# scverse/squidpy

Measured on AMD Instinct MI355X. Metric: nhood_enrichment permutations/sec (1e6 spots x 30 clusters), higher is better.
Workload: dtype u8 labels / u32 counts / i64 moments; 1 GPU; nhood_enrichment: 1000000 spots (1000x1000 hex grid, nnz=5992002), 30 clusters, 10000 permutations per step per GPU, on-device Philox-keyed label shuffles; collective=none

## Files before the change

squidpy_amd/csrc/sqgr_rng.h:

```cpp
#pragma once

#include <hip/hip_runtime.h>

#include <cstdint>

namespace sqgr {

constexpr uint32_t PHILOX_M0 = 0xD2511F53u, PHILOX_M1 = 0xCD9E8D57u;
constexpr uint32_t PHILOX_W0 = 0x9E3779B9u, PHILOX_W1 = 0xBB67AE85u;
constexpr uint32_t FEISTEL_C1 = 0x88B5u, FEISTEL_C2 = 0xDB2Du;
#ifndef SQGR_FEISTEL_ROUNDS
#define SQGR_FEISTEL_ROUNDS 8
#endif
constexpr int FEISTEL_ROUNDS = SQGR_FEISTEL_ROUNDS;

__host__ __device__ inline void philox4x32_10(uint32_t c[4], uint32_t k0, uint32_t k1) {
#pragma unroll
    for (int r = 0; r < 10; ++r) {
        uint64_t p0 = (uint64_t)PHILOX_M0 * c[0];
        uint64_t p1 = (uint64_t)PHILOX_M1 * c[2];
        uint32_t n0 = (uint32_t)(p1 >> 32) ^ c[1] ^ k0;
        uint32_t n1 = (uint32_t)p1;
        uint32_t n2 = (uint32_t)(p0 >> 32) ^ c[3] ^ k1;
        uint32_t n3 = (uint32_t)p0;
// ... 55 lines not shown
}

__host__ __device__ inline FeistelDomain make_domain(uint32_t n) {
    FeistelDomain d;
    d.n = n;
    const uint32_t r = isqrt_ceil(n);
    uint32_t a = 16u;
    while (a < r) a <<= 1;
    d.A = a;
    uint32_t b = (n + d.A - 1) / d.A;
    d.B = b < 16u ? 16u : b;
    uint32_t m = 1u;
    while (m < d.B) m <<= 1;
    d.Bmask = m - 1u;
    d.ash = 16u;
    for (uint32_t t = d.A; t > 1u; t >>= 1) --d.ash;
    d.bsh = 16u;
    for (uint32_t t = m; t > 1u; t >>= 1) --d.bsh;
    return d;
}

template <int NP>
__device__ __forceinline__ void feistel_rounds(u16x2 (&a)[NP], u16x2 (&b)[NP], const FeistelDomain& d,
                                               const uint32_t* const (&pk)[NP]) {
    const u16x2 am = (u16x2)((unsigned short)(d.A - 1u));
    const u16x2 ash = (u16x2)((unsigned short)d.ash), bsh = (u16x2)((unsigned short)d.bsh);
    const u16x2 BB = (u16x2)((unsigned short)d.B);
#pragma unroll
    for (int r = 0; r < FEISTEL_ROUNDS; r += 2) {
#pragma unroll
        for (int i = 0; i < NP; ++i) {
            const u16x2 k0 = __builtin_bit_cast(u16x2, pk[i][r]);
            a[i] = (a[i] + feistel_F2(b[i], k0, ash)) & am;
        }
#pragma unroll
        for (int i = 0; i < NP; ++i) {
            const u16x2 k1 = __builtin_bit_cast(u16x2, pk[i][r + 1]);
            u16x2 t = b[i] + feistel_F2(a[i], k1, bsh);
            t = __builtin_elementwise_min(t, (u16x2)(t - BB));
            b[i] = __builtin_elementwise_min(t, (u16x2)(t - BB));
        }
    }
}

template <int NP>
__device__ __forceinline__ void sigma_rounds(u16x2 (&a)[NP], u16x2 (&b)[NP], const FeistelDomain& d,
                                             const uint32_t* const (&pk)[NP]) {
    const u16x2 am = (u16x2)((unsigned short)(d.A - 1u));
    const u16x2 ash = (u16x2)((unsigned short)d.ash), bsh = (u16x2)((unsigned short)d.bsh);
    const u16x2 BB = (u16x2)((unsigned short)d.B);
#pragma unroll
    for (int i = 0; i < NP; ++i) {
        const u16x2 k0 = __builtin_bit_cast(u16x2, pk[i][0]);
        u16x2 t = b[i] + feistel_F2(a[i], k0, bsh);
        t = __builtin_elementwise_min(t, (u16x2)(t - BB));
        b[i] = __builtin_elementwise_min(t, (u16x2)(t - BB));
    }
#pragma unroll
    for (int i = 0; i < NP; ++i) {
        const u16x2 k1 = __builtin_bit_cast(u16x2, pk[i][1]);
        a[i] = (a[i] + feistel_F2(b[i], k1, ash)) & am;
    }
}

__host__ __device__ inline uint32_t grouped_perm(uint32_t x, const FeistelDomain& d, const uint32_t* gk, const uint32_t* sk) {
    uint32_t a = x / d.B, b = x - a * d.B;
    do {
        for (int r = 0; r < FEISTEL_ROUNDS; r += 2) {
            a = (a + feistel_F1(b, gk[r], d.ash)) & (d.A - 1u);
            uint32_t t = b + feistel_F1(a, gk[r + 1], d.bsh);
            t = t >= d.B ? t - d.B : t;
            b = t >= d.B ? t - d.B : t;
        }
    } while (a * d.B + b >= d.n);
    do {
        uint32_t t = b + feistel_F1(a, sk[0], d.bsh);
        t = t >= d.B ? t - d.B : t;
        b = t >= d.B ? t - d.B : t;
        a = (a + feistel_F1(b, sk[1], d.ash)) & (d.A - 1u);
    } while (a * d.B + b >= d.n);
    return a * d.B + b;
}

__host__ __device__ inline uint32_t feistel_perm(uint32_t x, const FeistelDomain& d, const uint32_t* rk) {
    uint32_t a = x / d.B, b = x - a * d.B;
    do {
        for (int r = 0; r < FEISTEL_ROUNDS; r += 2) {
            a = (a + feistel_F1(b, rk[r], d.ash)) & (d.A - 1u);
            uint32_t t = b + feistel_F1(a, rk[r + 1], d.bsh);
            t = t >= d.B ? t - d.B : t;
            b = t >= d.B ? t - d.B : t;
        }
        x = a * d.B + b;
    } while (x >= d.n);
    return x;
}

}
```

squidpy_amd/csrc/sqgr_shuffle.h:

```cpp
#pragma once
#include "sqgr_common.h"
#include "sqgr_pcg.h"
#include "sqgr_rng.h"

namespace sqgr {

__host__ __device__ constexpr int key_words_per_row(int B, int n_libs) {
    return n_libs * ((B / FEISTEL_GROUP) * 8 + (B / 2) * 2) < (B / 2) * 8 ? (B / 2) * 8 : n_libs * ((B / FEISTEL_GROUP) * 8 + (B / 2) * 2);
}

struct LibDom {
    FeistelDomain dom;
    uint32_t aoff;
};

__device__ __forceinline__ void slab_store16(uint8_t* __restrict__ batch_base, int64_t n, int64_t i, int pw, uint32_t w0, uint32_t w1,
                                             uint32_t w2, uint32_t w3) {
    if (pw == 16) {
        *reinterpret_cast<uint4*>(batch_base + (size_t)i * 16) = make_uint4(w0, w1, w2, w3);
    } else if (pw == 8) {
        *reinterpret_cast<uint2*>(batch_base + (size_t)i * 8) = make_uint2(w0, w1);
        *reinterpret_cast<uint2*>(batch_base + (size_t)n * 8 + (size_t)i * 8) = make_uint2(w2, w3);
    } else if (pw == 4) {
        uint32_t* d = reinterpret_cast<uint32_t*>(batch_base) + i;
        d[0] = w0; d[(size_t)n] = w1; d[(size_t)2 * n] = w2; d[(size_t)3 * n] = w3;
    } else if (pw == 2) {
        uint16_t* d = reinterpret_cast<uint16_t*>(batch_base) + i;
        const uint32_t w[4] = {w0, w1, w2, w3};
#pragma unroll
        for (int q = 0; q < 8; ++q) d[(size_t)q * n] = (uint16_t)(w[q >> 1] >> (16 * (q & 1)));
    } else {
        uint8_t* d = batch_base + i;
        const uint32_t w[4] = {w0, w1, w2, w3};
#pragma unroll
        for (int q = 0; q < 16; ++q) d[(size_t)q * n] = (uint8_t)(w[q >> 2] >> (8 * (q & 3)));
    }
}

int check_labels(const int32_t* labels, int64_t n, int K, bool allow_negative);

struct LabelShuffler {
    sqgr_ctx* ctx = nullptr;
    int64_t n = 0;
    int K = 0;
    int n_libs = 1;
    bool has_libs = false;
    LibDom dom0{};
    int blk_words = 0;
    DevBuf<uint32_t> cum;
    int kpad = 0;
    bool tab_lds = true;
    DevBuf<int32_t> lib_of, rank_of;
    DevBuf<LibDom> libs;
    DevBuf<uint8_t> base_pos;
    DevBuf<uint16_t> base16;
    DevBuf<int32_t> perm_idx;
    DevBuf<uint32_t> lib_off;
    DevBuf<int32_t> spot_of;
    PcgWorkspace pcg_ws;
    bool has_labels = false;
    int max_label_count = 0;
    bool wide() const { return K > 256; }
    bool mapped() const { return spot_of.p != nullptr; }

    static int create(sqgr_ctx* ctx, int64_t n, const int32_t* labels, int K, const int32_t* lib_ids, int n_libs, LabelShuffler* out);
    int independent_mode(int B, bool* independent) const;
    int keygen(const char* timer, uint64_t seed, int64_t perm0, int nrows, int B, bool independent, uint32_t* keys, hipStream_t st) const;
    int launch_shuffle_raw(int B, int nb, const uint32_t* keys, uint8_t* slab, hipStream_t st, bool independent, int pw = 16) const;
    int gather_labels16(const char* timer, int nb, int64_t p0, int64_t p_valid, uint16_t* slab16, hipStream_t st) const;
};

int label_shuffler_create(sqgr_ctx* ctx, int64_t n, const int32_t* labels, int K, LabelShuffler** out);
void label_shuffler_destroy(LabelShuffler* s);

int label_shuffler_philox(LabelShuffler* s, uint64_t seed, int64_t perm0, int nb, uint32_t* keys_ws, uint8_t* slab, hipStream_t st);

int label_shuffler_pcg64(LabelShuffler* s, const uint64_t* states_dev, int64_t pc, int64_t stride, uint8_t* W, hipStream_t st);

bool label_shuffler_wide(const LabelShuffler* s);
size_t label_shuffler_key_words16();
int label_shuffler_philox16(LabelShuffler* s, uint64_t seed, int64_t perm0, int nb, uint32_t* keys_ws, uint16_t* slab16, hipStream_t st);
int label_shuffler_pcg64_16(LabelShuffler* s, const uint64_t* states_dev, int64_t pc, uint16_t* slab16, hipStream_t st);

}
```

squidpy_amd/csrc/sqgr_shuffle.hip:

```cpp
#include "sqgr_shuffle.h"

#include <algorithm>
#include <cstdlib>

namespace sqgr {

__global__ void k_keygen(uint64_t seed, int64_t perm0, int nrows, int B, int n_libs, uint32_t* __restrict__ keys) {
    const int items = B / FEISTEL_GROUP + B / 2;
    const int64_t t = blockIdx.x * (int64_t)blockDim.x + threadIdx.x;
    if (t >= (int64_t)nrows * n_libs * items) return;
    const int item = (int)(t % items);
    const uint32_t lib = (uint32_t)((t / items) % n_libs);
    const int64_t row = t / ((int64_t)items * n_libs);
    uint32_t* out = keys + row * key_words_per_row(B, n_libs);
    const int64_t perm_row = perm0 + row * B;
    if (item < B / FEISTEL_GROUP) {
        uint32_t rk[8];
        group_keys(seed, (uint64_t)(perm_row / FEISTEL_GROUP + item), lib, rk);
#pragma unroll
        for (int i = 0; i < 8; ++i) out[((size_t)item * n_libs + lib) * 8 + i] = (rk[i] & 0xFFFFu) * 0x10001u;
    } else {
        const int tt = item - B / FEISTEL_GROUP;
        uint32_t ra[2], rb[2];
        sigma_keys(seed, (uint64_t)(perm_row + 2 * tt), lib, ra);
// ... 115 lines not shown
            }
            bool sentinel;
            if constexpr (SMALLK) {
                sentinel = ((word + sent_add) & 0x80808080u) != 0;
            } else {
                const uint32_t k = (uint32_t)K;
                sentinel = k > 255u || (word & 0xFFu) >= k || ((word >> 8) & 0xFFu) >= k || ((word >> 16) & 0xFFu) >= k || (word >> 24) >= k;
            }
            if (sentinel) {
#pragma unroll
                for (int j = 0; j < 4; ++j) {
                    if (K <= 255 && ((word >> (8 * j)) & 0xFFu) < (uint32_t)K) continue;
                    const int jj = j >> 1, sh = (j & 1) * 16;
                    const uint32_t* sk = ks + ((size_t)(w * 2 + jj) * n_libs + lib) * 2;
                    const uint32_t k0 = (sk[0] >> sh) & 0xFFFFu, k1 = (sk[1] >> sh) & 0xFFFFu;
                    uint32_t a = (apk[jj] >> sh) & 0xFFFFu, b = (bpk[jj] >> sh) & 0xFFFFu;
                    uint32_t x = a * dom.B + b;
                    while (x >= dom.n) {
                        uint32_t t = b + feistel_F1(a, k0, dom.bsh);
                        t = t >= dom.B ? t - dom.B : t;
                        b = t >= dom.B ? t - dom.B : t;
                        a = (a + feistel_F1(b, k1, dom.ash)) & (dom.A - 1u);
                        x = a * dom.B + b;
                    }
                    const uint32_t e = blk_at(a * 4u);
                    uint32_t l = (e & 0xFFFFu) + (b >= (e >> 16) ? 1u : 0u);
                    if (l >= (uint32_t)K) {
                        l = K <= 255 ? (e >> 8) & 0xFFu : 0u;
                        while (x >= tab[l]) ++l;
                    }
                    word = (word & ~(0xFFu << (8 * j))) | (l << (8 * j));
                }
            }
            out[w] = word;
        }
    };
    uint32_t outA[4], outB[4];
    emit_group((u16x2)(ga.x), (u16x2)(gb.x), ksA, outA);
    if (store1) emit_group((u16x2)(ga.y), (u16x2)(gb.y), ksB, outB);
    if constexpr (NG == 2) {
        uint4* dst = reinterpret_cast<uint4*>(slab_all + ((size_t)row0 * n + i) * B);
        dst[0] = make_uint4(outA[0], outA[1], outA[2], outA[3]);
        dst[1] = make_uint4(outB[0], outB[1], outB[2], outB[3]);
    } else {
        slab_store16(slab_all + (size_t)row0 * n * 16, n, i, pw, outA[0], outA[1], outA[2], outA[3]);
        if (store1) slab_store16(slab_all + (size_t)row1 * n * 16, n, i, pw, outB[0], outB[1], outB[2], outB[3]);
    }
    }
}

constexpr int SHUF_TAB_THREADS = 1024;
constexpr uint32_t SHUF_TAB_MAX_A = 1024;
constexpr int SHUF_TAB_BLOCKS_PER_CU = 20;
constexpr int SHUF_TAB_MIN_TRIPS = 16;
static_assert(SHUF_TAB_MAX_A * 4u <= (1u << 12), "k_shuffle_tab carries the high digit scaled by 4 in a 16-bit half: ash - 2 >= 4, a << 2 < 2^12");

__device__ __forceinline__ u16x2 shuf_tab_F2(u16x2 v, u16x2 k, u16x2 sh, u16x2 c1) {
    u16x2 x = v * c1 + k;
    x ^= x >> (u16x2)(7);
    x *= (u16x2)(FEISTEL_C2);
    return x >> sh;
}
__device__ __forceinline__ void shuf_tab_rounds(u16x2& a, u16x2& b, const uint32_t (&kp)[8], u16x2 am, u16x2 ash, u16x2 bsh, u16x2 BB,
                                                u16x2 c1) {
#pragma unroll
    for (int r = 0; r < FEISTEL_ROUNDS; r += 2) {
        a = (a + shuf_tab_F2(b, __builtin_bit_cast(u16x2, kp[r]), ash, c1)) & am;
        u16x2 t = b + shuf_tab_F2(a, __builtin_bit_cast(u16x2, kp[r + 1]), bsh, c1);
        t = __builtin_elementwise_min(t, (u16x2)(t - BB));
        b = __builtin_elementwise_min(t, (u16x2)(t - BB));
    }
}
__device__ __forceinline__ uint32_t first_label(uint32_t e, uint32_t bpk, uint32_t zero) {
    uint32_t word;
    asm("v_cmp_le_u32_sdwa vcc, %1, %2 src0_sel:WORD_1 src1_sel:WORD_0\n\t"
        "v_addc_co_u32_sdwa %0, vcc, %1, %3, vcc dst_sel:BYTE_0 dst_unused:UNUSED_PAD src0_sel:BYTE_0 src1_sel:DWORD\n\t"
        "s_nop 0"
        : "=v"(word)
        : "v"(e), "v"(bpk), "v"(zero)
        : "vcc");
    return word;
}

template <bool SMALLK, bool NOMAP>
__global__ __launch_bounds__(SHUF_TAB_THREADS, 8) void k_shuffle_tab(int64_t n, const uint32_t* __restrict__ cum, int kpad, int blk_words, int K,
                                                                  const uint32_t* __restrict__ keys, LibDom dom0, int nrows,
                                                                  uint8_t* __restrict__ slab_all, int pw, const int32_t* __restrict__ spot_of,
                                                                  int tab_word0) {
    extern __shared__ uint32_t s_lds[];
    uint32_t* s_cum = s_lds + blk_words;
    for (int t = threadIdx.x; t < kpad; t += SHUF_TAB_THREADS) s_cum[t] = cum[t];
    for (int t = threadIdx.x; t < blk_words; t += SHUF_TAB_THREADS) s_lds[t] = cum[kpad + t];
    const FeistelDomain dom = dom0.dom;
    const int row0 = 2 * blockIdx.y;
    const int row1 = min(row0 + 1, nrows - 1);
    const bool store1 = row0 + 1 < nrows;
    constexpr size_t row_words = key_words_per_row(16, 1);
    const uint32_t* kgA = keys + (size_t)row0 * row_words;
    const uint32_t* kgB = keys + (size_t)row1 * row_words;
    const uint32_t* ksA = kgA + 8;
    const uint32_t* ksB = kgB + 8;
    const u16x2 BB = (u16x2)((unsigned short)dom.B);
    {
        const u16x2 bsh = (u16x2)((unsigned short)dom.bsh);
        const int words = (int)dom.A * 8;
        for (int idx = threadIdx.x; idx < words; idx += SHUF_TAB_THREADS) {
            const u16x2 av = (u16x2)((unsigned short)(idx >> 3));
            const int t = idx & 7;
            u16x2 fa = feistel_F2(av, __builtin_bit_cast(u16x2, ksA[t * 2]), bsh);
            u16x2 fb = feistel_F2(av, __builtin_bit_cast(u16x2, ksB[t * 2]), bsh);
            fa = __builtin_elementwise_min(fa, (u16x2)(fa - BB));
            fb = __builtin_elementwise_min(fb, (u16x2)(fb - BB));
            s_lds[tab_word0 + idx] = __builtin_bit_cast(uint32_t, fa);
            s_lds[tab_word0 + words + idx] = __builtin_bit_cast(uint32_t, fb);
        }
    }
    __syncthreads();
    const uint32_t zero = 0;
    const uint32_t sent_add = (uint32_t)(128 - K) * 0x01010101u;
    const uint32_t* tab = s_cum + 1;
    typedef __attribute__((address_space(3))) const uint32_t lds_word;
    typedef uint32_t u32x4 __attribute__((ext_vector_type(4)));
    typedef __attribute__((address_space(3))) const u32x4 lds_row;
    auto blk_at = [&](uint32_t byte_off) { return *reinterpret_cast<lds_word*>((uintptr_t)byte_off); };
    const uint32_t tabA = (uint32_t)tab_word0 * 4u, tabB = tabA + dom.A * 32u;
    const u16x2 am = (u16x2)((unsigned short)(dom.A - 1u));
    const u16x2 ash = (u16x2)((unsigned short)dom.ash), bsh = (u16x2)((unsigned short)dom.bsh);
    const u16x2 am4 = (u16x2)((unsigned short)((dom.A - 1u) << 2));
    const u16x2 ash4 = (u16x2)((unsigned short)(dom.ash - 2u));
    uint32_t c1w = FEISTEL_C1 * 0x10001u;
    asm volatile("" : "+v"(c1w));
    const u16x2 c1 = __builtin_bit_cast(u16x2, c1w);
    const uint32_t n32 = (uint32_t)n, stride = gridDim.x * (uint32_t)SHUF_TAB_THREADS;
    uint32_t i = blockIdx.x * (uint32_t)SHUF_TAB_THREADS + threadIdx.x;
    uint32_t sa = 0, sb = 0, a0 = 0, b0 = 0;
    if constexpr (NOMAP) {
        sa = stride / dom.B;
        sb = stride - sa * dom.B;
        asm volatile("" : "+v"(sa), "+v"(sb));
        a0 = i / dom.B;
        b0 = i - a0 * dom.B;
    }
    uint32_t kp[8];
#pragma unroll
    for (int r = 0; r < 8; ++r) {
        kp[r] = (kgA[r] & 0xFFFFu) | (kgB[r] & 0xFFFF0000u);
        asm volatile("" : "+v"(kp[r]));
    }
    for (; i < n32; i += stride) {
    if constexpr (!NOMAP) {
        const uint32_t x0 = (uint32_t)spot_of[i];
        a0 = x0 / dom.B;
        b0 = x0 - a0 * dom.B;
    }
    u16x2 ga = (u16x2)((unsigned short)a0), gb = (u16x2)((unsigned short)b0);
    {
        shuf_tab_rounds(ga, gb, kp, am, ash, bsh, BB, c1);
        bool need0 = __umul24((uint32_t)ga.x, dom.B) + (uint32_t)gb.x >= dom.n;
        bool need1 = __umul24((uint32_t)ga.y, dom.B) + (uint32_t)gb.y >= dom.n;
        while (__builtin_expect(need0 | need1, 0)) {
            u16x2 na = ga, nb = gb;
            shuf_tab_rounds(na, nb, kp, am, ash, bsh, BB, c1);
            if (need0) { ga.x = na.x; gb.x = nb.x; }
            if (need1) { ga.y = na.y; gb.y = nb.y; }
            need0 = __umul24((uint32_t)ga.x, dom.B) + (uint32_t)gb.x >= dom.n;
            need1 = __umul24((uint32_t)ga.y, dom.B) + (uint32_t)gb.y >= dom.n;
        }
    }
    if constexpr (NOMAP) {
        a0 += sa;
        b0 += sb;
        if (b0 >= dom.B) { b0 -= dom.B; ++a0; }
    }
    auto emit_group = [&](const uint32_t ga1, const uint32_t gb1, const uint32_t row_off, const uint32_t* ks, uint32_t (&out)[4]) {
        const u16x2 gsa4 = (u16x2)((unsigned short)(ga1 << 2)), gsb = (u16x2)((unsigned short)gb1);
        const u32x4 r0 = *reinterpret_cast<lds_row*>((uintptr_t)row_off);
        const u32x4 r1 = *reinterpret_cast<lds_row*>((uintptr_t)(row_off + 16u));
        const uint32_t f1[8] = {r0.x, r0.y, r0.z, r0.w, r1.x, r1.y, r1.z, r1.w};
#pragma unroll
        for (int w = 0; w < FEISTEL_GROUP / 4; ++w) {
            uint32_t word;
            uint32_t a4pk[2], bpk[2];
#pragma unroll
            for (int jj = 0; jj < 2; ++jj) {
                const u16x2 t = gsb + __builtin_bit_cast(u16x2, f1[w * 2 + jj]);
                const u16x2 b = __builtin_elementwise_min(t, (u16x2)(t - BB));
                const u16x2 k1 = __builtin_bit_cast(u16x2, ks[(w * 2 + jj) * 2 + 1]);
                bpk[jj] = __builtin_bit_cast(uint32_t, b);
                a4pk[jj] = __builtin_bit_cast(uint32_t, (u16x2)((gsa4 + shuf_tab_F2(b, k1, ash4, c1)) & am4));
                const uint32_t e0 = blk_at(a4pk[jj] & 0xFFFFu);
                const uint32_t e1 = blk_at(a4pk[jj] >> 16);
                if (jj == 0) {
                    word = first_label(e0, bpk[jj], zero);
                    put_label<1, 1>(word, e1, bpk[jj], zero);
                } else {
                    put_label<2, 0>(word, e0, bpk[jj], zero);
                    put_label<3, 1>(word, e1, bpk[jj], zero);
                }
            }
            bool sentinel;
            if constexpr (SMALLK) {
                sentinel = ((word + sent_add) & 0x80808080u) != 0;
            } else {
                const uint32_t k = (uint32_t)K;
                sentinel = k > 255u || (word & 0xFFu) >= k || ((word >> 8) & 0xFFu) >= k || ((word >> 16) & 0xFFu) >= k || (word >> 24) >= k;
            }
            if (sentinel) {
#pragma unroll
                for (int j = 0; j < 4; ++j) {
                    if (K <= 255 && ((word >> (8 * j)) & 0xFFu) < (uint32_t)K) continue;
                    const int jj = j >> 1, sh = (j & 1) * 16;
                    const uint32_t* sk = ks + (w * 2 + jj) * 2;
                    uint32_t a = ((a4pk[jj] >> sh) & 0xFFFFu) >> 2, b = (bpk[jj] >> sh) & 0xFFFFu;
                    uint32_t x = a * dom.B + b;
                    if (x >= dom.n) {
                        const uint32_t k0 = (sk[0] >> sh) & 0xFFFFu, k1 = (sk[1] >> sh) & 0xFFFFu;
                        do {
                            uint32_t t = b + feistel_F1(a, k0, dom.bsh);
                            t = t >= dom.B ? t - dom.B : t;
                            b = t >= dom.B ? t - dom.B : t;
                            a = (a + feistel_F1(b, k1, dom.ash)) & (dom.A - 1u);
                            x = a * dom.B + b;
                        } while (x >= dom.n);
                    }
                    const uint32_t e = blk_at(a * 4u);
                    uint32_t l = (e & 0xFFFFu) + (b >= (e >> 16) ? 1u : 0u);
                    if (l >= (uint32_t)K) {
                        l = K <= 255 ? (e >> 8) & 0xFFu : 0u;
                        while (x >= tab[l]) ++l;
                    }
                    word = (word & ~(0xFFu << (8 * j))) | (l << (8 * j));
                }
            }
            out[w] = word;
        }
    };
    uint32_t outA[4], outB[4];
    emit_group((uint32_t)ga.x, (uint32_t)gb.x, tabA + (uint32_t)ga.x * 32u, ksA, outA);
    if (store1) emit_group((uint32_t)ga.y, (uint32_t)gb.y, tabB + (uint32_t)ga.y * 32u, ksB, outB);
    slab_store16(slab_all + (size_t)row0 * n * 16, n, i, pw, outA[0], outA[1], outA[2], outA[3]);
    if (store1) slab_store16(slab_all + (size_t)row1 * n * 16, n, i, pw, outB[0], outB[1], outB[2], outB[3]);
    }
}

template <bool SMALLK>
__global__ __launch_bounds__(256) void k_shuffle_indep(int64_t n, const uint32_t* __restrict__ cum, int kpad, int blk_words, int K,
                                                       const uint32_t* __restrict__ keys, LibDom dom0, uint8_t* __restrict__ slab_all, int pw) {
    extern __shared__ uint32_t s_lds[];
    uint32_t* s_cum = s_lds + blk_words;
    for (int t = threadIdx.x; t < kpad; t += 256) s_cum[t] = cum[t];
    for (int t = threadIdx.x; t < blk_words; t += 256) s_lds[t] = cum[kpad + t];
    __syncthreads();
    const int row = blockIdx.y;
    const uint32_t* krow = keys + (size_t)row * key_words_per_row(16, 1);
    const uint32_t zero = 0;
    const uint32_t sent_add = (uint32_t)(128 - K) * 0x01010101u;
    const FeistelDomain dom = dom0.dom;
    const uint32_t* tab = s_cum + 1;
    typedef __attribute__((address_space(3))) const uint32_t lds_word;
    auto blk_at = [&](uint32_t byte_off) { return *reinterpret_cast<lds_word*>((uintptr_t)byte_off); };
    for (int64_t i = blockIdx.x * (int64_t)blockDim.x + threadIdx.x; i < n; i += (int64_t)gridDim.x * blockDim.x) {
        const uint32_t x0 = (uint32_t)i;
        const uint32_t a0 = x0 / dom.B, b0 = x0 - a0 * dom.B;
        uint32_t out[4];
#pragma unroll
        for (int w = 0; w < 4; ++w) {
            uint32_t word = 0, apk[2], bpk[2];
#pragma unroll
            for (int jj = 0; jj < 2; ++jj) {
                const uint32_t* const pk[1] = {krow + (w * 2 + jj) * 8};
                u16x2 ga = (u16x2)((unsigned short)a0), gb = (u16x2)((unsigned short)b0);
                bool need0 = true, need1 = true;
                do {
                    u16x2 na[1] = {ga}, nb[1] = {gb};
                    feistel_rounds<1>(na, nb, dom, pk);
                    if (need0) { ga.x = na[0].x; gb.x = nb[0].x; }
                    if (need1) { ga.y = na[0].y; gb.y = nb[0].y; }
                    need0 = __umul24((uint32_t)ga.x, dom.B) + (uint32_t)gb.x >= dom.n;
                    need1 = __umul24((uint32_t)ga.y, dom.B) + (uint32_t)gb.y >= dom.n;
                } while (need0 | need1);
                apk[jj] = __builtin_bit_cast(uint32_t, ga);
                bpk[jj] = __builtin_bit_cast(uint32_t, gb);
                const uint32_t a4 = apk[jj] << 2;
                const uint32_t e0 = blk_at(a4 & 0xFFFFu);
                const uint32_t e1 = blk_at(a4 >> 16);
                if (jj == 0) {
                    put_label<0, 0>(word, e0, bpk[jj], zero);
                    put_label<1, 1>(word, e1, bpk[jj], zero);
                } else {
                    put_label<2, 0>(word, e0, bpk[jj], zero);
                    put_label<3, 1>(word, e1, bpk[jj], zero);
                }
            }
            bool sentinel;
            if constexpr (SMALLK) {
                sentinel = ((word + sent_add) & 0x80808080u) != 0;
            } else {
                const uint32_t k = (uint32_t)K;
                sentinel = k > 255u || (word & 0xFFu) >= k || ((word >> 8) & 0xFFu) >= k || ((word >> 16) & 0xFFu) >= k || (word >> 24) >= k;
            }
            if (sentinel) {
#pragma unroll
                for (int j = 0; j < 4; ++j) {
                    if (K <= 255 && ((word >> (8 * j)) & 0xFFu) < (uint32_t)K) continue;
                    const int jj = j >> 1, sh = (j & 1) * 16;
                    const uint32_t a = (apk[jj] >> sh) & 0xFFFFu, b = (bpk[jj] >> sh) & 0xFFFFu;
                    const uint32_t x = a * dom.B + b;
                    const uint32_t e = blk_at(a * 4u);
                    uint32_t l = (e & 0xFFFFu) + (b >= (e >> 16) ? 1u : 0u);
                    if (l >= (uint32_t)K) {
                        l = K <= 255 ? (e >> 8) & 0xFFu : 0u;
                        while (x >= tab[l]) ++l;
                    }
                    word = (word & ~(0xFFu << (8 * j))) | (l << (8 * j));
                }
            }
            out[w] = word;
        }
        slab_store16(slab_all + (size_t)row * n * 16, n, i, pw, out[0], out[1], out[2], out[3]);
    }
}

template <bool HAS_LIBS>
__global__ __launch_bounds__(256) void k_shuffle16(int64_t n, const uint32_t* __restrict__ cum, int kpad, int blk_words, int K,
                                                   const uint32_t* __restrict__ keys, LibDom dom0, int n_libs,
// ... 113 lines not shown
    p->n = n;
    p->K = K;
    const bool libs_on = lib_ids && n_libs >= 1;
    p->has_libs = libs_on;
    p->n_libs = libs_on ? n_libs : 1;
    p->kpad = K + 1;
    std::vector<int64_t> cnt((size_t)p->n_libs, 0);
    std::vector<uint32_t> hist((size_t)p->n_libs * K, 0);
    std::vector<int32_t> rank;
    if (libs_on) rank.resize((size_t)n);
    for (int64_t i = 0; i < n; ++i) {
        int l = 0;
        if (libs_on) {
            l = lib_ids[i];
            SQGR_REQUIRE(l >= 0 && l < n_libs, "lib_ids[%lld]=%d outside [0,%d)", (long long)i, l, n_libs);
            rank[i] = (int32_t)cnt[l];
        }
        cnt[l]++;
        if (labels) hist[(size_t)l * K + labels[i]]++;
    }
    if (labels) {
        for (int k = 0; k < K; ++k) {
            int64_t tot = 0;
            for (int l = 0; l < p->n_libs; ++l) tot += hist[(size_t)l * K + k];
            p->max_label_count = (int)std::max<int64_t>(p->max_label_count, tot);
        }
    }
    std::vector<uint32_t> cum((size_t)p->n_libs * p->kpad, 0xFFFFFFFFu);
    std::vector<LibDom> doms((size_t)p->n_libs);
    size_t blk_total = 0;
    for (int l = 0; l < p->n_libs; ++l) {
        uint32_t run = 0;
        for (int k = 0; k < K; ++k) {
            cum[(size_t)l * p->kpad + k] = run;
            run += hist[(size_t)l * K + k];
        }
        doms[l].dom = make_domain((uint32_t)(cnt[l] > 0 ? cnt[l] : 1));
        doms[l].aoff = (uint32_t)blk_total;
        blk_total += doms[l].dom.A;
    }
    p->blk_words = (int)blk_total;
    p->tab_lds = (size_t)p->n_libs * p->kpad * 4 + blk_total * 4 <= 150 * 1024;
    if (!p->tab_lds && (K <= 256 || blk_total * 4 > 150 * 1024)) {
        set_error("library/label tables (%zu bytes) exceed the LDS budget of the shuffle kernel",
                  (size_t)p->n_libs * p->kpad * 4 + blk_total * 4);
        return SQGR_ERR_UNSUPPORTED;
    }
    std::vector<uint32_t> blk(blk_total, 0);
    for (int l = 0; l < p->n_libs; ++l) {
        const uint32_t* c = &cum[(size_t)l * p->kpad];
        const uint64_t n_l = (uint64_t)cnt[l];
        const uint32_t SENT = (uint32_t)K | (0xFFFFu << 16);
        uint32_t lab = 0;
        for (uint32_t a = 0; a < doms[l].dom.A; ++a) {
            const uint64_t lo = (uint64_t)a * doms[l].dom.B, hi = lo + doms[l].dom.B;
            uint32_t word;
            if (lo >= n_l) {
                word = SENT;
            } else {
                while (lab + 1 < (uint32_t)K && c[lab + 1] <= lo) ++lab;
                const uint64_t end = hi < n_l ? hi : n_l;
                uint32_t events = 0, ev_label = 0;
                uint64_t ev_pos = 0;
                for (uint32_t k2 = lab + 1; k2 < (uint32_t)K && c[k2] < end; ++k2) {
                    const uint64_t nxt = k2 + 1 < (uint32_t)K ? c[k2 + 1] : n_l;
                    if (c[k2] >= nxt) continue;
                    if (events == 0) { ev_label = k2; ev_pos = c[k2] - lo; }
                    ++events;
                }
                if (hi > n_l) {
                    if (events == 0) { ev_label = (uint32_t)K; ev_pos = n_l - lo; }
                    ++events;
                }
                if (events == 0)
                    word = lab | (0xFFFFu << 16);
                else if (events == 1 && ev_label == lab + 1 && ev_pos > 0)
                    word = lab | ((uint32_t)ev_pos << 16);
                else
                    word = SENT | (K <= 255 ? lab << 8 : 0u);
            }
            blk[doms[l].aoff + a] = word;
        }
    }
    cum.insert(cum.end(), blk.begin(), blk.end());
    p->dom0.dom = make_domain((uint32_t)n);
    p->dom0.aoff = 0;
    if (!libs_on) p->dom0 = doms[0];
    {
        std::vector<uint32_t> off((size_t)p->n_libs + 1, 0);
        for (int l = 0; l < p->n_libs; ++l) off[l + 1] = off[l] + (uint32_t)cnt[l];
        std::vector<uint8_t> base((size_t)n, 0);
        if (labels)
            for (int64_t i = 0; i < n; ++i) base[libs_on ? off[lib_ids[i]] + (uint32_t)rank[i] : (uint32_t)i] = (uint8_t)labels[i];
        p->has_labels = labels != nullptr;
        if (K > 256 && labels) {
            std::vector<uint16_t> b16((size_t)n, 0);
            for (int64_t i = 0; i < n; ++i) b16[libs_on ? off[lib_ids[i]] + (uint32_t)rank[i] : (uint32_t)i] = (uint16_t)labels[i];
            SQGR_TRY(p->base16.alloc((size_t)n));
            if (hipMemcpy(p->base16.p, b16.data(), (size_t)n * 2, hipMemcpyHostToDevice) != hipSuccess) return SQGR_ERR_HIP;
        }
        SQGR_TRY(p->base_pos.alloc((size_t)n));
        SQGR_TRY(p->lib_off.alloc(off.size()));
        hipError_t e2 = hipMemcpy(p->base_pos.p, base.data(), (size_t)n, hipMemcpyHostToDevice);
        if (e2 == hipSuccess) e2 = hipMemcpy(p->lib_off.p, off.data(), off.size() * 4, hipMemcpyHostToDevice);
        if (e2 != hipSuccess) {
            set_error("label upload failed: %s", hipGetErrorString(e2));
            return SQGR_ERR_HIP;
        }
    }
    SQGR_TRY(p->cum.alloc(cum.size()));
    hipError_t e = hipMemcpy(p->cum.p, cum.data(), cum.size() * 4, hipMemcpyHostToDevice);
    if (e == hipSuccess && libs_on) {
        SQGR_TRY(p->lib_of.alloc((size_t)n));
        SQGR_TRY(p->rank_of.alloc((size_t)n));
        SQGR_TRY(p->libs.alloc((size_t)n_libs));
        e = hipMemcpy(p->lib_of.p, lib_ids, (size_t)n * 4, hipMemcpyHostToDevice);
        if (e == hipSuccess) e = hipMemcpy(p->rank_of.p, rank.data(), (size_t)n * 4, hipMemcpyHostToDevice);
        if (e == hipSuccess) e = hipMemcpy(p->libs.p, doms.data(), (size_t)n_libs * sizeof(LibDom), hipMemcpyHostToDevice);
    }
    if (e != hipSuccess) {
        set_error("label upload failed: %s", hipGetErrorString(e));
        return SQGR_ERR_HIP;
    }
    return SQGR_OK;
}

int LabelShuffler::independent_mode(int B, bool* independent) const {
    const char* e = getenv("SQGR_SHUFFLE_INDEPENDENT");
    *independent = e && atoi(e) == 1;
    SQGR_REQUIRE(!*independent || (B == 16 && !has_libs && !wide()), "SQGR_SHUFFLE_INDEPENDENT needs 16-wide rows, K <= 256 and no libraries");
    return SQGR_OK;
}

int LabelShuffler::keygen(const char* timer, uint64_t seed, int64_t perm0, int nrows, int B, bool independent, uint32_t* keys,
                          hipStream_t st) const {
    if (timer) {
        LaunchTimer t(ctx, timer, st);
        return keygen(nullptr, seed, perm0, nrows, B, independent, keys, st);
    }
    const int64_t nk = (int64_t)nrows * n_libs * (B / FEISTEL_GROUP + B / 2);
    if (independent) k_keygen_indep<<<(unsigned)ceil_div((int64_t)nrows * 8, 256), 256, 0, st>>>(seed, perm0, nrows, keys);
    else k_keygen<<<(unsigned)ceil_div(nk, 256), 256, 0, st>>>(seed, perm0, nrows, B, n_libs, keys);
    SQGR_HIP(hipGetLastError());
    return SQGR_OK;
}

int LabelShuffler::launch_shuffle_raw(int B, int nb, const uint32_t* keys, uint8_t* slab, hipStream_t st, bool independent, int pw) const {
    unsigned gx = (unsigned)ceil_div(n, 256);
    int per_cu = 96;
    const char* env_blocks = getenv("SQGR_SHUFFLE_BLOCKS_PER_CU");
    if (env_blocks && atoi(env_blocks) > 0) per_cu = atoi(env_blocks);
    gx = std::min<unsigned>(gx, (unsigned)(per_cu * std::max(ctx->cu_count, 1)) / (unsigned)std::max(nb, 1) + 1);
    LaunchTimer t(ctx, wide() ? "nhood_shuffle16" : "nhood_shuffle", st);
    const size_t lds = (tab_lds ? (size_t)n_libs * kpad * 4 : 0) + (size_t)blk_words * 4;
    if (wide()) {
        if (B != 16) {
            set_error("more than 256 clusters: 16 permutations per pass only");
            return SQGR_ERR_UNSUPPORTED;
        }
        uint16_t* slab16 = reinterpret_cast<uint16_t*>(slab);
        if (has_libs) {
            SQGR_TRY(allow_lds(k_shuffle16<true>, lds));
            k_shuffle16<true><<<dim3(gx, nb), 256, lds, st>>>(n, cum.p, kpad, blk_words, K, keys, dom0, n_libs, lib_of.p,
                                                              rank_of.p, libs.p, slab16, tab_lds ? 1 : 0);
        } else {
            SQGR_TRY(allow_lds(k_shuffle16<false>, lds));
            k_shuffle16<false><<<dim3(gx, nb), 256, lds, st>>>(n, cum.p, kpad, blk_words, K, keys, dom0, n_libs, lib_of.p,
                                                               rank_of.p, libs.p, slab16, tab_lds ? 1 : 0);
        }
        SQGR_HIP(hipGetLastError());
        return SQGR_OK;
    }
    if (independent) {
        if (B != 16 || has_libs) {
            set_error("SQGR_SHUFFLE_INDEPENDENT: 16 permutations per row and no libraries only");
            return SQGR_ERR_UNSUPPORTED;
        }
        if (K <= 126) k_shuffle_indep<true><<<dim3(gx, nb), 256, lds, st>>>(n, cum.p, kpad, blk_words, K, keys, dom0, slab, pw);
        else k_shuffle_indep<false><<<dim3(gx, nb), 256, lds, st>>>(n, cum.p, kpad, blk_words, K, keys, dom0, slab, pw);
        SQGR_HIP(hipGetLastError());
        return SQGR_OK;
    }
    const unsigned gy = (unsigned)(B == 32 ? nb : (nb + 1) / 2);
    {
        const char* env_tab = getenv("SQGR_SHUFFLE_TABLE");
        const int mode = env_tab ? atoi(env_tab) : -1;
        const uint32_t A = dom0.dom.A;
        const size_t tab_word0 = (lds / 4 + 7) & ~(size_t)7;
        const size_t lds_tab = tab_word0 * 4 + (size_t)2 * A * 32;
        const char* why = nullptr;
        if (B != 16) why = "32 permutations per row";
        else if (has_libs) why = "libraries (per-library domains and keys)";
        else if (A > SHUF_TAB_MAX_A) why = "more than 2^20 spots (high digit A > 1024: the two tables exceed 64 KB)";
        else if (lds_tab > LDS_BUDGET / 2) why = "tables do not fit two blocks per CU";
        if (mode == 2 && why) {
            set_error("SQGR_SHUFFLE_TABLE=2: the table kernel does not take this input: %s", why);
            return SQGR_ERR_UNSUPPORTED;
        }
        const int cus = std::max(ctx->cu_count, 1);
        const int64_t block_trips = ceil_div(n, SHUF_TAB_THREADS) * (int64_t)gy;
        const bool big = block_trips >= (int64_t)SHUF_TAB_MIN_TRIPS * 2 * cus;
        if (!why && mode != 0 && (mode == 1 || mode == 2 || big)) {
            int tab_per_cu = SHUF_TAB_BLOCKS_PER_CU;
            if (env_blocks && atoi(env_blocks) > 0) tab_per_cu = atoi(env_blocks);
            const unsigned nblk = (unsigned)ceil_div(n, SHUF_TAB_THREADS);
            const unsigned cap = (unsigned)(tab_per_cu * cus) / gy + 1;
            const unsigned trips = (nblk + cap - 1) / cap;
            const unsigned tx = (nblk + trips - 1) / trips;
#define SQGR_SHUFFLE_TAB(SK, NOMAP)                                                                                             \
    do {                                                                                                                       \
        SQGR_TRY(allow_lds(k_shuffle_tab<SK, NOMAP>, lds_tab));                                                                \
        k_shuffle_tab<SK, NOMAP><<<dim3(tx, gy), SHUF_TAB_THREADS, lds_tab, st>>>(n, cum.p, kpad, blk_words, K, keys, dom0, nb, \
                                                                                slab, pw, spot_of.p, (int)tab_word0);        \
    } while (0)
            if (K <= 126) {
                if (spot_of.p) SQGR_SHUFFLE_TAB(true, false); else SQGR_SHUFFLE_TAB(true, true);
            } else {
                if (spot_of.p) SQGR_SHUFFLE_TAB(false, false); else SQGR_SHUFFLE_TAB(false, true);
            }
#undef SQGR_SHUFFLE_TAB
            SQGR_HIP(hipGetLastError());
            return SQGR_OK;
        }
    }
#define SQGR_SHUFFLE(BB, LIBS, SK)                                                                                             \
    k_shuffle<BB, LIBS, SK><<<dim3(gx, gy), 256, lds, st>>>(n, cum.p, kpad, blk_words, K, keys, dom0, n_libs, nb, \
                                                            lib_of.p, rank_of.p, libs.p, slab, pw, spot_of.p)
#define SQGR_SHUFFLE_K(BB, LIBS) \
    if (K <= 126) SQGR_SHUFFLE(BB, LIBS, true); else SQGR_SHUFFLE(BB, LIBS, false)
    if (B == 32) {
        if (has_libs) { SQGR_SHUFFLE_K(32, true); } else { SQGR_SHUFFLE_K(32, false); }
    } else {
        if (has_libs) { SQGR_SHUFFLE_K(16, true); } else { SQGR_SHUFFLE_K(16, false); }
    }
#undef SQGR_SHUFFLE_K
#undef SQGR_SHUFFLE
    SQGR_HIP(hipGetLastError());
    return SQGR_OK;
}

int LabelShuffler::gather_labels16(const char* timer, int nb, int64_t p0, int64_t p_valid, uint16_t* slab16, hipStream_t st) const {
    LaunchTimer t(ctx, timer, st);
    k_gather_labels16<<<dim3((unsigned)ceil_div(n, 256), nb), 256, 0, st>>>(n, base16.p, perm_idx.p, p0, p_valid, slab16);
    SQGR_HIP(hipGetLastError());
    return SQGR_OK;
}

int label_shuffler_create(sqgr_ctx* ctx, int64_t n, const int32_t* labels, int K, LabelShuffler** out) {
    SQGR_REQUIRE(ctx && labels && out && n > 0, "ctx/labels/out is NULL or n <= 0");
    *out = nullptr;
    LabelShuffler* s = new LabelShuffler();
    const int rc = LabelShuffler::create(ctx, n, labels, K, nullptr, 0, s);
    if (rc != SQGR_OK) {
        delete s;
        return rc;
    }
    *out = s;
    return SQGR_OK;
}

void label_shuffler_destroy(LabelShuffler* s) { delete s; }

bool label_shuffler_wide(const LabelShuffler* s) { return s->wide(); }

size_t label_shuffler_key_words16() { return (size_t)key_words_per_row(16, 1); }

int label_shuffler_philox16(LabelShuffler* s, uint64_t seed, int64_t perm0, int nb, uint32_t* keys_ws, uint16_t* slab16, hipStream_t st) {
    if (!s->wide() || perm0 % FEISTEL_GROUP != 0) {
        set_error("label_shuffler_philox16: needs more than 256 labels and perm0 (%lld) a multiple of %d", (long long)perm0, FEISTEL_GROUP);
        return SQGR_ERR_INVALID;
    }
    SQGR_TRY(s->keygen("ligrec_keygen", seed, perm0, nb, 16, false, keys_ws, st));
    return s->launch_shuffle_raw(16, nb, keys_ws, reinterpret_cast<uint8_t*>(slab16), st, false);
}

int label_shuffler_pcg64_16(LabelShuffler* s, const uint64_t* states_dev, int64_t pc, uint16_t* slab16, hipStream_t st) {
    if (!s->wide() || !s->base16.p) {
        set_error("label_shuffler_pcg64_16: needs more than 256 labels");
        return SQGR_ERR_INVALID;
    }
    const int64_t n = s->n;
    SQGR_TRY(s->perm_idx.ensure((size_t)pc * n));
    SQGR_TRY(pcg_permutations_dev(s->ctx, s->pcg_ws, n, states_dev, pc, s->perm_idx.p, st));
    return s->gather_labels16("ligrec_gather_labels16", (int)ceil_div(pc, 16), 0, pc, slab16, st);
}

int label_shuffler_philox(LabelShuffler* s, uint64_t seed, int64_t perm0, int nb, uint32_t* keys_ws, uint8_t* slab,
                          hipStream_t st) {
    if (perm0 % FEISTEL_GROUP != 0) {
        set_error("label_shuffler_philox: perm0=%lld is not a multiple of %d", (long long)perm0, FEISTEL_GROUP);
        return SQGR_ERR_INVALID;
    }
    SQGR_TRY(s->keygen("ligrec_keygen", seed, perm0, nb, 32, false, keys_ws, st));
    return s->launch_shuffle_raw(32, nb, keys_ws, slab, st, false);
}

int label_shuffler_pcg64(LabelShuffler* s, const uint64_t* states_dev, int64_t pc, int64_t stride, uint8_t* W, hipStream_t st) {
    return pcg_shuffle_labels(s->ctx, s->pcg_ws, s->n, 1, s->lib_off.p, s->base_pos.p, states_dev, pc, stride, W, st, "ligrec_pcg64_shuffle");
}

}
```

Before: 1.253 million permutations/s.

## Drop sentinel checks in table shuffle, fix out-of-range spots with inverse Feistel

Adds a FIX variant of the table shuffle kernel. Out-of-domain blocks are mapped to label K-1, so the per-word sentinel/cycle-walk branch is never taken. A small follow-up kernel then handles the few padding slots: it inverts the Feistel rounds to find which spot landed on each padding value and rewrites that spot's label correctly. This removes divergent cycle-walking from the hot loop, at the cost of an extra launch, scattered byte writes, and eligibility checks done on the host.

```diff
diff --git a/squidpy_amd/csrc/sqgr_rng.h b/squidpy_amd/csrc/sqgr_rng.h
--- a/squidpy_amd/csrc/sqgr_rng.h
+++ b/squidpy_amd/csrc/sqgr_rng.h
@@ -161,6 +161,22 @@
     return a * d.B + b;
 }
 
+__host__ __device__ inline uint32_t feistel_unadd_b(uint32_t b, uint32_t a, uint32_t k, const FeistelDomain& d) {
+    uint32_t f = feistel_F1(a, k, d.bsh);
+    f = f >= d.B ? f - d.B : f;
+    return b >= f ? b - f : b + d.B - f;
+}
+__host__ __device__ inline void sigma_inverse(uint32_t& a, uint32_t& b, const FeistelDomain& d, uint32_t k0, uint32_t k1) {
+    a = (a - feistel_F1(b, k1, d.ash)) & (d.A - 1u);
+    b = feistel_unadd_b(b, a, k0, d);
+}
+__host__ __device__ inline void feistel_rounds_inverse(uint32_t& a, uint32_t& b, const FeistelDomain& d, const uint32_t* rk) {
+    for (int r = FEISTEL_ROUNDS - 2; r >= 0; r -= 2) {
+        b = feistel_unadd_b(b, a, rk[r + 1], d);
+        a = (a - feistel_F1(b, rk[r], d.ash)) & (d.A - 1u);
+    }
+}
+
 __host__ __device__ inline uint32_t feistel_perm(uint32_t x, const FeistelDomain& d, const uint32_t* rk) {
     uint32_t a = x / d.B, b = x - a * d.B;
     do {
diff --git a/squidpy_amd/csrc/sqgr_shuffle.h b/squidpy_amd/csrc/sqgr_shuffle.h
--- a/squidpy_amd/csrc/sqgr_shuffle.h
+++ b/squidpy_amd/csrc/sqgr_shuffle.h
@@ -37,6 +37,30 @@
     }
 }
 
+__host__ __device__ inline size_t slab_label_offset(int64_t n, int64_t i, int pw, int j) {
+    return (size_t)(j / pw) * (size_t)n * pw + (size_t)i * pw + (size_t)(j % pw);
+}
+
+__host__ __device__ inline bool shuffle_fix_target(uint32_t y, const FeistelDomain& d, const uint32_t* gk, uint32_t k0, uint32_t k1,
+                                                   uint32_t* spot, uint32_t* rank_out) {
+    const uint32_t ya = y / d.B, yb = y - ya * d.B;
+    uint32_t a = ya, b = yb;
+    sigma_inverse(a, b, d, k0, k1);
+    if (a * d.B + b >= d.n) return false;
+    do feistel_rounds_inverse(a, b, d, gk); while (a * d.B + b >= d.n);
+    *spot = a * d.B + b;
+    a = ya;
+    b = yb;
+    do {
+        uint32_t t = b + feistel_F1(a, k0, d.bsh);
+        t = t >= d.B ? t - d.B : t;
+        b = t >= d.B ? t - d.B : t;
+        a = (a + feistel_F1(b, k1, d.ash)) & (d.A - 1u);
+    } while (a * d.B + b >= d.n);
+    *rank_out = a * d.B + b;
+    return true;
+}
+
 int check_labels(const int32_t* labels, int64_t n, int K, bool allow_negative);
 
 struct LabelShuffler {
@@ -60,6 +84,7 @@
     PcgWorkspace pcg_ws;
     bool has_labels = false;
     int max_label_count = 0;
+    const char* fix_why = nullptr;
     bool wide() const { return K > 256; }
     bool mapped() const { return spot_of.p != nullptr; }
 
diff --git a/squidpy_amd/csrc/sqgr_shuffle.hip b/squidpy_amd/csrc/sqgr_shuffle.hip
--- a/squidpy_amd/csrc/sqgr_shuffle.hip
+++ b/squidpy_amd/csrc/sqgr_shuffle.hip
@@ -221,15 +221,22 @@
     return word;
 }
 
-template <bool SMALLK, bool NOMAP>
+template <bool SMALLK, bool NOMAP, bool FIX>
 __global__ __launch_bounds__(SHUF_TAB_THREADS, 8) void k_shuffle_tab(int64_t n, const uint32_t* __restrict__ cum, int kpad, int blk_words, int K,
                                                                   const uint32_t* __restrict__ keys, LibDom dom0, int nrows,
                                                                   uint8_t* __restrict__ slab_all, int pw, const int32_t* __restrict__ spot_of,
                                                                   int tab_word0) {
+    static_assert(!FIX || (SMALLK && NOMAP), "the FIX pair runs without a spot map and with K <= 126 only");
     extern __shared__ uint32_t s_lds[];
     uint32_t* s_cum = s_lds + blk_words;
-    for (int t = threadIdx.x; t < kpad; t += SHUF_TAB_THREADS) s_cum[t] = cum[t];
-    for (int t = threadIdx.x; t < blk_words; t += SHUF_TAB_THREADS) s_lds[t] = cum[kpad + t];
+    if constexpr (FIX) {
+        const int past = (int)((uint32_t)n / dom0.dom.B);
+        for (int t = threadIdx.x; t < blk_words; t += SHUF_TAB_THREADS)
+            s_lds[t] = t >= past ? ((uint32_t)(K - 1) | (0xFFFFu << 16)) : cum[kpad + t];
+    } else {
+        for (int t = threadIdx.x; t < kpad; t += SHUF_TAB_THREADS) s_cum[t] = cum[t];
+        for (int t = threadIdx.x; t < blk_words; t += SHUF_TAB_THREADS) s_lds[t] = cum[kpad + t];
+    }
     const FeistelDomain dom = dom0.dom;
     const int row0 = 2 * blockIdx.y;
     const int row1 = min(row0 + 1, nrows - 1);
@@ -338,7 +345,9 @@
                 }
             }
             bool sentinel;
-            if constexpr (SMALLK) {
+            if constexpr (FIX) {
+                sentinel = false;
+            } else if constexpr (SMALLK) {
                 sentinel = ((word + sent_add) & 0x80808080u) != 0;
             } else {
                 const uint32_t k = (uint32_t)K;
@@ -380,6 +389,26 @@
     slab_store16(slab_all + (size_t)row0 * n * 16, n, i, pw, outA[0], outA[1], outA[2], outA[3]);
     if (store1) slab_store16(slab_all + (size_t)row1 * n * 16, n, i, pw, outB[0], outB[1], outB[2], outB[3]);
     }
+}
+
+__global__ __launch_bounds__(256) void k_shuffle_fix(int64_t n, const uint32_t* __restrict__ cum, int K, const uint32_t* __restrict__ keys,
+                                                     FeistelDomain dom, int nrows, uint32_t E, uint8_t* __restrict__ slab_all, int pw) {
+    const int64_t t = blockIdx.x * (int64_t)blockDim.x + threadIdx.x;
+    if (t >= (int64_t)nrows * FEISTEL_GROUP * E) return;
+    const uint32_t e = (uint32_t)(t % E);
+    const int j = (int)((t / E) % FEISTEL_GROUP);
+    const int64_t row = t / ((int64_t)E * FEISTEL_GROUP);
+    const uint32_t* krow = keys + (size_t)row * key_words_per_row(16, 1);
+    const uint32_t* sk = krow + 8 + (j >> 1) * 2;
+    const int sh = (j & 1) * 16;
+    uint32_t spot, x;
+    if (!shuffle_fix_target(dom.n + e, dom, krow, (sk[0] >> sh) & 0xFFFFu, (sk[1] >> sh) & 0xFFFFu, &spot, &x)) return;
+    uint32_t lo = 0, hi = (uint32_t)K - 1u;
+    while (lo < hi) {
+        const uint32_t mid = (lo + hi) >> 1;
+        if (x < cum[mid + 1]) hi = mid; else lo = mid + 1;
+    }
+    slab_all[(size_t)row * n * 16 + slab_label_offset(n, spot, pw, j)] = (uint8_t)lo;
 }
 
 template <bool SMALLK>
@@ -659,6 +688,20 @@
             blk[doms[l].aoff + a] = word;
         }
     }
+    if (libs_on) {
+        p->fix_why = "libraries (per-library domains and keys)";
+    } else if (K > 126) {
+        p->fix_why = "more than 126 clusters";
+    } else {
+        const FeistelDomain& d = doms[0].dom;
+        const uint32_t past = (uint32_t)n / d.B;
+        for (uint32_t a = 0; a < past && a < d.A && !p->fix_why; ++a)
+            if ((blk[a] & 0xFFu) == (uint32_t)K)
+                p->fix_why = "a block of the label-sorted base has several label starts or skips an empty category (lab0 = K)";
+        const uint32_t tail = (uint32_t)n - past * d.B;
+        if (!p->fix_why && tail > 0 && blk[past] != ((uint32_t)(K - 1) | (tail << 16)))
+            p->fix_why = "the block that reaches past the last rank does not end in label K - 1 in two-field form";
+    }
     cum.insert(cum.end(), blk.begin(), blk.end());
     p->dom0.dom = make_domain((uint32_t)n);
     p->dom0.aoff = 0;
@@ -728,8 +771,14 @@
     const char* env_blocks = getenv("SQGR_SHUFFLE_BLOCKS_PER_CU");
     if (env_blocks && atoi(env_blocks) > 0) per_cu = atoi(env_blocks);
     gx = std::min<unsigned>(gx, (unsigned)(per_cu * std::max(ctx->cu_count, 1)) / (unsigned)std::max(nb, 1) + 1);
+    const char* env_fix = getenv("SQGR_SHUFFLE_FIX");
+    const int fix_mode = env_fix ? atoi(env_fix) : -1;
+    if (fix_mode == 2 && (wide() || independent)) {
+        set_error("SQGR_SHUFFLE_FIX=2: the launch is not eligible: %s", wide() ? "more than 126 clusters" : "SQGR_SHUFFLE_INDEPENDENT=1");
+        return SQGR_ERR_UNSUPPORTED;
+    }
     LaunchTimer t(ctx, wide() ? "nhood_shuffle16" : "nhood_shuffle", st);
-    const size_t lds = (tab_lds ? (size_t)n_libs * kpad * 4 : 0) + (size_t)blk_words * 4;
+    const size_t lds =(tab_lds ? (size_t)n_libs * kpad * 4 : 0) + (size_t)blk_words * 4;
     if (wide()) {
         if (B != 16) {
             set_error("more than 256 clusters: 16 permutations per pass only");
@@ -777,26 +826,40 @@
         const int cus = std::max(ctx->cu_count, 1);
         const int64_t block_trips = ceil_div(n, SHUF_TAB_THREADS) * (int64_t)gy;
         const bool big = block_trips >= (int64_t)SHUF_TAB_MIN_TRIPS * 2 * cus;
-        if (!why && mode != 0 && (mode == 1 || mode == 2 || big)) {
+        const char* fix_no = why ? why : mode == 0 ? "SQGR_SHUFFLE_TABLE=0" : spot_of.p ? "a spot map (the rank is not the slab row)" : fix_why;
+        if (fix_mode == 2 && fix_no) {
+            set_error("SQGR_SHUFFLE_FIX=2: the launch is not eligible: %s", fix_no);
+            return SQGR_ERR_UNSUPPORTED;
+        }
+        const bool fix = fix_mode != 0 && !fix_no;
+        if (!why && mode != 0 && (mode == 1 || mode == 2 || big || fix_mode == 2)) {
             int tab_per_cu = SHUF_TAB_BLOCKS_PER_CU;
             if (env_blocks && atoi(env_blocks) > 0) tab_per_cu = atoi(env_blocks);
             const unsigned nblk = (unsigned)ceil_div(n, SHUF_TAB_THREADS);
             const unsigned cap = (unsigned)(tab_per_cu * cus) / gy + 1;
             const unsigned trips = (nblk + cap - 1) / cap;
             const unsigned tx = (nblk + trips - 1) / trips;
-#define SQGR_SHUFFLE_TAB(SK, NOMAP)                                                                                             \
-    do {                                                                                                                       \
-        SQGR_TRY(allow_lds(k_shuffle_tab<SK, NOMAP>, lds_tab));                                                                \
-        k_shuffle_tab<SK, NOMAP><<<dim3(tx, gy), SHUF_TAB_THREADS, lds_tab, st>>>(n, cum.p, kpad, blk_words, K, keys, dom0, nb, \
-                                                                                slab, pw, spot_of.p, (int)tab_word0);        \
+#define SQGR_SHUFFLE_TAB(SK, NOMAP, FIX)                                                                                            \
+    do {                                                                                                                           \
+        SQGR_TRY(allow_lds(k_shuffle_tab<SK, NOMAP, FIX>, lds_tab));                                                               \
+        k_shuffle_tab<SK, NOMAP, FIX><<<dim3(tx, gy), SHUF_TAB_THREADS, lds_tab, st>>>(n, cum.p, kpad, blk_words, K, keys, dom0, nb, \
+                                                                                     slab, pw, spot_of.p, (int)tab_word0);       \
     } while (0)
-            if (K <= 126) {
-                if (spot_of.p) SQGR_SHUFFLE_TAB(true, false); else SQGR_SHUFFLE_TAB(true, true);
+            if (fix) {
+                SQGR_SHUFFLE_TAB(true, true, true);
+            } else if (K <= 126) {
+                if (spot_of.p) SQGR_SHUFFLE_TAB(true, false, false); else SQGR_SHUFFLE_TAB(true, true, false);
             } else {
-                if (spot_of.p) SQGR_SHUFFLE_TAB(false, false); else SQGR_SHUFFLE_TAB(false, true);
+                if (spot_of.p) SQGR_SHUFFLE_TAB(false, false, false); else SQGR_SHUFFLE_TAB(false, true, false);
             }
 #undef SQGR_SHUFFLE_TAB
             SQGR_HIP(hipGetLastError());
+            const uint32_t E = A * dom0.dom.B - (uint32_t)n;
+            if (fix && E > 0) {
+                const int64_t threads = (int64_t)nb * FEISTEL_GROUP * E;
+                k_shuffle_fix<<<(unsigned)ceil_div(threads, 256), 256, 0, st>>>(n, cum.p, K, keys, dom0.dom, nb, E, slab, pw);
+                SQGR_HIP(hipGetLastError());
+            }
             return SQGR_OK;
         }
     }
```

Result: faster. 1.292 million permutations/s (median of 6 runs) (+3.1%).
